# tomershay100/mp3-steganography-lib

Measured on AMD Instinct MI355X. Metric: MP3 frames/sec (decode+re-encode) @44.1kHz stereo 128kbps, 1→8 GPU, higher is better.
Workload: dtype f64 (decode) / int32 (encode); 1 GPU; 10000-frame full decode->stego-embed->re-encode pipeline per MI355X (BASELINE configs[2]); MP3 main data + side info resident in HBM, MP3 frames out; the message cursor chain is decided and the serial chains of the rate loop are checked on the device inside every step; frames_per_gpu=10000, channels=2, message_bits=536, chain_verdict_units_to_redo=0, message_variant_entries=1874, parallelism=frames sharded over 1 GPU(s), no collective

## Files before the change

### mp3-steganography-lib_amd/csrc/k_decode_stream.hpp

```cpp
#pragma once
#ifndef MP3S_ST_CLOCKS
#define MP3S_ST_CLOCKS 0
#endif
#if MP3S_ST_CLOCKS
__device__ uint32_t g_st_clocks[4096 * 8];
extern "C" __attribute__((visibility("default"))) int mp3s_debug_st_clocks(uint32_t *out)
{
    (void)hipDeviceSynchronize();
    return (int)hipMemcpyFromSymbol(out, HIP_SYMBOL(g_st_clocks), sizeof(uint32_t) * 4096 * 8);
}
#endif

namespace mp3s {

constexpr int ST_WAVES = 4;
constexpr int ST_P43_N = 512;

struct StShared {
    double pow2q[POW2Q_N];
    double pow2h[POW2H_N];
    uint32_t side[ST_WAVES][2][18];
    double exp2f[ST_WAVES][2][64];
    double exp1f[ST_WAVES][2][4];
    double win[4][36];
    double tail[ST_WAVES][18][64];
    double p43[2 * ST_P43_N];
    double cx[16][32], wt[16][32];
};

__device__ __forceinline__ double st_requant_line(const DevTables &tab, StShared &sh, int wave, const int16_t *__restrict__ is, int g, int c, int sr, int s)
{
    const uint8_t *gb = reinterpret_cast<const uint8_t *>(sh.side[wave][c]);
    const int bt = gb[2] & 3, mixed = gb[3] ? 1 : 0;
    const int cse = bt == 2 ? 1 : (mixed ? 2 : 0);
    const int sbs = (s * 3641) >> 16;
    const uint32_t m = tab.rq_map[sr][cse][sbs][s - 18 * sbs];
    const int x = is[((long)g * 2 + c) * 576 + s];
    uint32_t ax = (uint32_t)(x < 0 ? -x : x);
    ax = ax < (uint32_t)POW43_N ? ax : (uint32_t)(POW43_N - 1);
    const double a = tab.pow43[ax];
    const double sa = x < 0 ? -a : a;
    return (sa * sh.exp1f[wave][c][m >> 6]) * sh.exp2f[wave][c][m & 63];
}

__device__ __forceinline__ double st_row_dot16(double t, const double (&c)[16])
{
    double x = 0.0;
    asm("s_nop 4\n\t"
        "v_fmac_f64_dpp %0, %1, %2 row_newbcast:0 row_mask:0xf bank_mask:0xf\n\t"
        "v_fmac_f64_dpp %0, %1, %3 row_newbcast:1 row_mask:0xf bank_mask:0xf\n\t"
        "v_fmac_f64_dpp %0, %1, %4 row_newbcast:2 row_mask:0xf bank_mask:0xf\n\t"
        "v_fmac_f64_dpp %0, %1, %5 row_newbcast:3 row_mask:0xf bank_mask:0xf\n\t"
        "v_fmac_f64_dpp %0, %1, %6 row_newbcast:4 row_mask:0xf bank_mask:0xf\n\t"
        "v_fmac_f64_dpp %0, %1, %7 row_newbcast:5 row_mask:0xf bank_mask:0xf\n\t"
        "v_fmac_f64_dpp %0, %1, %8 row_newbcast:6 row_mask:0xf bank_mask:0xf\n\t"
        "v_fmac_f64_dpp %0, %1, %9 row_newbcast:7 row_mask:0xf bank_mask:0xf\n\t"
        "v_fmac_f64_dpp %0, %1, %10 row_newbcast:8 row_mask:0xf bank_mask:0xf\n\t"
        "v_fmac_f64_dpp %0, %1, %11 row_newbcast:9 row_mask:0xf bank_mask:0xf\n\t"
        "v_fmac_f64_dpp %0, %1, %12 row_newbcast:10 row_mask:0xf bank_mask:0xf\n\t"
        "v_fmac_f64_dpp %0, %1, %13 row_newbcast:11 row_mask:0xf bank_mask:0xf\n\t"
        "v_fmac_f64_dpp %0, %1, %14 row_newbcast:12 row_mask:0xf bank_mask:0xf\n\t"
        "v_fmac_f64_dpp %0, %1, %15 row_newbcast:13 row_mask:0xf bank_mask:0xf\n\t"
        "v_fmac_f64_dpp %0, %1, %16 row_newbcast:14 row_mask:0xf bank_mask:0xf\n\t"
        "v_fmac_f64_dpp %0, %1, %17 row_newbcast:15 row_mask:0xf bank_mask:0xf"
        : "+v"(x)
        : "v"(t), "v"(c[0]), "v"(c[1]), "v"(c[2]), "v"(c[3]), "v"(c[4]), "v"(c[5]), "v"(c[6]), "v"(c[7]), "v"(c[8]), "v"(c[9]), "v"(c[10]),
          "v"(c[11]), "v"(c[12]), "v"(c[13]), "v"(c[14]), "v"(c[15]));
    return x;
}

template <int NCH, bool F32, bool MARGIN = false>
__global__ __launch_bounds__(ST_WAVES * 64, 2) void k_dec_stream(
    const int16_t *__restrict__ is, const mp3s_granule_si *__restrict__ si, const mp3s_frame_hdr *__restrict__ hdr,
    int n_granules, int run, int n_halo, void *__restrict__ pcm_out, int sf_base, double eps_scale,
    uint2 *__restrict__ fix_list, int32_t *__restrict__ fix_count,
    double *__restrict__ mg_x = nullptr, double *__restrict__ mg_eps = nullptr, long mg_base = 0, long mg_cap = 0)
{
    __shared__ StShared sh;
    const int wave = __builtin_amdgcn_readfirstlane(threadIdx.x >> 6), lane = threadIdx.x & 63;
#if MP3S_ST_CLOCKS
    const unsigned long long ck_start = __builtin_readcyclecounter();
    unsigned long long ck_req = 0, ck_rows = 0, ck_syn = 0, ck_setup = 0;
#endif
    for (int i = threadIdx.x; i < POW2Q_N; i += blockDim.x) sh.pow2q[i] = c_tab.pow2q[i];
    if (threadIdx.x < POW2H_N) sh.pow2h[threadIdx.x] = c_tab.pow2h[threadIdx.x];
    if (threadIdx.x < 144) (&sh.win[0][0])[threadIdx.x] = (&c_tab.sine_block[0][0])[threadIdx.x];
    for (int i = threadIdx.x; i < 2 * ST_P43_N; i += blockDim.x) {
        const int x = i - ST_P43_N;
        sh.p43[i] = x < 0 ? -c_tab.pow43[-x] : c_tab.pow43[x];
    }
    for (int i = threadIdx.x; i < 512; i += blockDim.x) {
        sh.cx[i >> 5][i & 31] = c_tab.stream_cx[i & 31][i >> 5];
        sh.wt[i >> 5][i & 31] = c_tab.stream_taps[F32 ? 0 : 1][i & 31][i >> 5];
    }
    __syncthreads();
    const int ga = (xcd_tile() * ST_WAVES + wave) * run;
    if (ga >= n_granules) return;

    const int ch = lane >> 5, sb = lane & 31;
    const bool live = ch < NCH;
    const uint32_t sgn_odd = (sb & 1) ? 0x80000000u : 0u;
    auto flip = [&](double x) { return __hiloint2double(__double2hiint(x) ^ (int)sgn_odd, __double2loint(x)); };
    int addr_a, addr_b;
    {
        const int ka = sb <= 15 ? 16 + sb : (sb == 16 ? 0 : 48 - sb);
        const int kb = sb <= 15 ? 16 - sb : sb - 16;
        auto holder = [&](int k) { return (ch << 5) + ((k & 1) ? (k >> 1) : 16 + (k >> 1)); };
        addr_a = holder(ka) * 4; addr_b = holder(kb) * 4;
    }
    const uint32_t sgn_lo = sb < 16 ? 0x80000000u : 0u;
    const double eps_k = (2.0 * c_tab.synth_eps_a + c_tab.synth_eps_g + 2.0 * c_tab.synth_eps_x * c_tab.synth_xbound) * eps_scale;
    const double xb_k = 2.0 * c_tab.synth_xbound;
    const long halo_slots = (long)n_halo * 36;
    typedef double __attribute__((address_space(3))) lds_f64;
    lds_f64 *const tl = (lds_f64 *)reinterpret_cast<double *>(&sh.tail[wave][0][lane]);

    double acc[18];
#pragma unroll
    for (int i = 0; i < 18; i++) acc[i] = 0.0;
    double gm1 = 0.0, gm2 = 0.0;
    const int s_a = [&] { const uint32_t sf = hdr[ga >> 1].stream_first; return sf > (uint32_t)sf_base ? (int)(sf - (uint32_t)sf_base) * 2 : 0; }();
    bool fresh = true;
    GranIn next_in = {};
    bool have_next = false;

    const int gi0 = ga - 2 >= s_a ? -2 : (ga - 1 >= s_a ? -1 : 0);
    mp3s_frame_hdr fh = hdr[(ga + gi0) >> 1];
    int sr_map = fh.sr_idx < 3 ? fh.sr_idx : 0;
    uint32_t mwl[5];
#pragma unroll
    for (int k = 0; k < 5; k++) mwl[k] = reinterpret_cast<const uint32_t *>(c_tab.rq_map[sr_map][0][sb])[k];
#if MP3S_ST_CLOCKS
    ck_setup = __builtin_readcyclecounter() - ck_start;
#endif
#pragma unroll 1
    for (int gi = gi0; gi < run; gi++) {
        const int g = ga + gi;
        if (g >= n_granules) break;
#if MP3S_ST_CLOCKS
        const unsigned long long ck_a = __builtin_readcyclecounter();
#endif
        const int first_gran = fh.stream_first > (uint32_t)sf_base ? (int)(fh.stream_first - (uint32_t)sf_base) * 2 : 0;
        const int sr = fh.sr_idx < 3 ? fh.sr_idx : 0;
        const bool ms = fh.ms_stereo != 0;
        fh = hdr[(g + 1 < n_granules ? g + 1 : g) >> 1];
        if (g == first_gran) fresh = true;
        if (fresh) {
#pragma unroll
            for (int i = 0; i < 18; i++) { tl[i * 64] = 0.0; acc[i] = 0.0; }
            gm1 = gm2 = 0.0;
            fresh = false;
        }
        const bool tail_only = gi == -2;
        const bool emit = gi >= 0;
        int zoff = 0;
        asm volatile("" : "+s"(zoff));
        const DevTables &tab = *reinterpret_cast<const DevTables *>(reinterpret_cast<const char *>(&c_tab) + zoff);
        const double(*C12)[6] = tab.imdct_cos12;

        double v[18];
        int bt, cse;
        const GranIn in = have_next ? next_in : dec_fetch(is, si, g, NCH, lane);
        bool quick;
        uint32_t w0, w1;
        {
            const uint32_t d0a = (uint32_t)__builtin_amdgcn_readlane((int)in.side, 0), d1a = (uint32_t)__builtin_amdgcn_readlane((int)in.side, 1);
            const uint32_t d0b = (uint32_t)__builtin_amdgcn_readlane((int)in.side, 18), d1b = (uint32_t)__builtin_amdgcn_readlane((int)in.side, 19);
            auto is_long = [](uint32_t d0) { return ((d0 >> 16) & 3u) != 2u && (d0 >> 24) == 0u; };
            quick = is_long(d0a) && (NCH == 1 || is_long(d0b));
            w0 = ch ? d0b : d0a; w1 = ch ? d1b : d1a;
            uint32_t hi_bits = 0;
#pragma unroll
            for (int k = 0; k < 9; k++) {
                uint32_t t;
                asm("v_pk_add_u16 %0, %1, %2" : "=v"(t) : "v"(in.xw[k]), "v"(0x02000200u));
                hi_bits |= t;
            }
            quick = quick && __ballot((hi_bits & 0xfc00fc00u) != 0) == 0;
        }
        if (quick && sr != sr_map) {
            sr_map = sr;
#pragma unroll
            for (int k = 0; k < 5; k++) mwl[k] = reinterpret_cast<const uint32_t *>(tab.rq_map[sr][0][sb])[k];
        }
        if (quick) {
            bt = (int)((w0 >> 16) & 3u); cse = 0;
            const int gg = (int)(w0 & 0xffu), mult2 = ((w0 >> 8) & 0xffu) ? 2 : 1, preflag = (w1 & 0xffu) ? 1 : 0;
            double *e2 = sh.exp2f[wave][ch];
            const int bsrc = ((ch ? 18 : 0) + 2 + (sb >> 2)) * 4;
            const uint32_t sfw = (uint32_t)__builtin_amdgcn_ds_bpermute(bsrc, (int)in.side);
            if (sb < 22) {
                const int pt = sb < 11 || sb > 20 ? 0 : (int)((0x2333221111ull >> ((sb - 11) * 4)) & 15);
                const int k2 = mult2 * ((int)((sfw >> ((sb & 3) * 8)) & 15u) + preflag * pt);
                e2[sb] = sh.pow2h[k2 < POW2H_N ? k2 : POW2H_N - 1];
            }
            const double e1 = sh.pow2q[gg - 210 - POW2Q_MIN];
            __builtin_amdgcn_s_waitcnt(0xc07f);
            __builtin_amdgcn_wave_barrier();
#pragma unroll
            for (int k = 0; k < 18; k++) {
                const uint32_t xwk = in.xw[k >> 1];
                const int x = (k & 1) ? (int)xwk >> 16 : (int)(int16_t)xwk;
                const double sa = sh.p43[x + ST_P43_N];
                uint32_t i2;
                asm("v_bfe_u32 %0, %1, %2, 6" : "=v"(i2) : "v"(mwl[k >> 2]), "n"((k & 3) * 8));
                v[k] = (sa * e1) * e2[i2];
            }
            if (ms && NCH == 2) {
#pragma unroll
                for (int k = 0; k < 18; k++) {
                    const double o = shfl_xor_f64(v[k], 32);
                    v[k] = ch == 0 ? (v[k] + o) / tab.sqrt2 : (o - v[k]) / tab.sqrt2;
                }
            }
        } else {
            const uint32_t sd0a = (uint32_t)__builtin_amdgcn_readlane((int)in.side, 0), sd0b = (uint32_t)__builtin_amdgcn_readlane((int)in.side, 18);
            auto case_of = [](uint32_t d0) { return ((d0 >> 16) & 3u) == 2u ? 1 : ((d0 >> 24) ? 2 : 0); };
            const int cse_a = case_of(sd0a), cse_b = NCH == 2 ? case_of(sd0b) : cse_a;
            if (cse_a == cse_b && cse_a != 0) {
                dec_requant_tables(sh, wave, in, NCH, lane, bt, cse);
                const uint32_t *srcw = reinterpret_cast<const uint32_t *>(tab.reorder_src[sr] + sb * 18);
                uint32_t sw[9];
#pragma unroll
                for (int k = 0; k < 9; k++) sw[k] = srcw[k];
#pragma unroll
                for (int k = 0; k < 18; k++) {
                    const int s = (int)(int16_t)(sw[k >> 1] >> ((k & 1) * 16));
                    v[k] = s >= 0 && live ? st_requant_line(tab, sh, wave, is, g, ch, sr, s) : 0.0;
                }
                if (ms && NCH == 2) {
#pragma unroll
                    for (int k = 0; k < 18; k++) {
                        const double o = shfl_xor_f64(v[k], 32);
                        v[k] = ch == 0 ? (v[k] + o) / tab.sqrt2 : (o - v[k]) / tab.sqrt2;
                    }
                }
                cse = -1;
            } else
                dec_requant_ms(tab, sh, wave, v, in, sr, ms, NCH, lane, bt, cse);
        }
        if (cse > 0) {
            const uint32_t *srcw = reinterpret_cast<const uint32_t *>(tab.reorder_src[sr] + sb * 18);
            uint32_t sw[9];
#pragma unroll
            for (int k = 0; k < 9; k++) sw[k] = srcw[k];
#pragma unroll
            for (int k = 0; k < 18; k++) {
                const int s = (int)(int16_t)(sw[k >> 1] >> ((k & 1) * 16));
                double x = 0.0;
                if (s >= 0 && live) {
                    x = st_requant_line(tab, sh, wave, is, g, ch, sr, s);
                    if (ms && NCH == 2) {
                        const double o = st_requant_line(tab, sh, wave, is, g, ch ^ 1, sr, s);
                        x = ch == 0 ? (x + o) / tab.sqrt2 : (o - x) / tab.sqrt2;
                    }
                }
                v[k] = x;
            }
        } else if (cse == 0) {
#pragma unroll
            for (int i = 0; i < 8; i++) {
                const double nlo = dpp_f64<0x138>(v[17 - i]);
                const double nhi = dpp_f64<0x130>(v[i]);
                const double cs = tab.alias_cs[i], ca = tab.alias_ca[i];
                const double lo = v[i] * cs + nlo * ca;
                const double hi = v[17 - i] * cs - nhi * ca;
                v[i] = sb >= 1 ? lo : v[i];
                v[17 - i] = sb <= 30 ? hi : v[17 - i];
            }
        }
        double eps_t = 0.0;
        bool safe = true;
        if (!F32) {
            double s = 0.0;
#pragma unroll
            for (int k = 0; k < 18; k++) s += fabs(v[k]);
            s += dpp_f64<0xB1>(s);
            s += dpp_f64<0x4E>(s);
            s += dpp_f64<0x141>(s);
            s += dpp_f64<0x140>(s);
            const double o = __hiloint2double(__builtin_amdgcn_ds_swizzle(__double2hiint(s), 0x401f), __builtin_amdgcn_ds_swizzle(__double2loint(s), 0x401f));
            const double gc = s + o;
            double gx = gc > gm1 ? gc : gm1;
            gx = gx > gm2 ? gx : gm2;
            if (!(gx >= 0.0)) gx = __builtin_inf();
            eps_t = eps_k * gx;
            safe = __ballot(!(xb_k * gx < 2147483000.0)) == 0;
            gm2 = gm1; gm1 = gc;
        }

#if MP3S_ST_CLOCKS
        const unsigned long long ck_b = __builtin_readcyclecounter();
        ck_req += ck_b - ck_a;
#endif
        double S[18];
        if (bt != 2) {
            const double *wl = sh.win[bt];
            double p[9], q[9];
            {
                const Row18s r = load_row18s(tab.imdct_rot, 0);
#pragma unroll
                for (int k = 0; k < 9; k++) {
                    const double c = 2 * k < 8 ? r.a[2 * k] : (2 * k < 16 ? r.b[2 * k - 8] : r.c[2 * k - 16]);
                    const double sn = 2 * k + 1 < 8 ? r.a[2 * k + 1] : (2 * k + 1 < 16 ? r.b[2 * k + 1 - 8] : r.c[2 * k + 1 - 16]);
                    p[k] = __builtin_fma(v[17 - k], sn, v[k] * c);
                    q[k] = __builtin_fma(v[17 - k], c, -(v[k] * sn));
                }
            }
            struct StageIn { Row18s c; double w[4], t[4]; };
            auto stage_in = [&](auto mc) {
                constexpr int m = decltype(mc)::value;
                StageIn in;
                in.c = load_row18s(tab.imdct_pq, m);
#pragma unroll
                for (int h = 0; h < 2; h++) {
                    const int n = h == 0 ? 2 * m : 2 * m - 1;
                    in.w[2 * h] = in.w[2 * h + 1] = in.t[2 * h] = in.t[2 * h + 1] = 0.0;
                    if (n < 0 || n > 17) continue;
                    if (n >= 9) {
                        const int i = n - 9;
                        in.w[2 * h] = wl[i]; in.w[2 * h + 1] = wl[17 - i];
                        in.t[2 * h] = tl[i * 64]; in.t[2 * h + 1] = tl[(17 - i) * 64];
                    } else {
                        const int i = 26 - n;
                        in.w[2 * h] = wl[i]; in.w[2 * h + 1] = wl[53 - i];
                    }
                }
                return in;
            };
            auto stage = [&](auto mc, const StageIn &in) {
                constexpr int m = decltype(mc)::value;
                double P = 0.0, Q = 0.0;
#pragma unroll
                for (int k = 0; k < 9; k++) {
                    const double cp = k < 8 ? in.c.a[k] : in.c.b[0];
                    const double cq = k < 7 ? in.c.b[1 + k] : in.c.c[k - 7];
                    if (m != 9) P = __builtin_fma(p[k], cp, P);
                    if (m != 0) Q = __builtin_fma(q[k], cq, Q);
                }
#pragma unroll
                for (int h = 0; h < 2; h++) {
                    const int n = h == 0 ? 2 * m : 2 * m - 1;
                    if (n < 0 || n > 17) continue;
                    const double y = h == 0 ? P + Q : P - Q;
                    if (n >= 9) {
                        const int i = n - 9;
                        double xa = y * in.w[2 * h] + in.t[2 * h];
                        double xb = -y * in.w[2 * h + 1] + in.t[2 * h + 1];
                        if (i & 1) xa = flip(xa);
                        if ((17 - i) & 1) xb = flip(xb);
                        S[i] = xa; S[17 - i] = xb;
                    } else {
                        const int i = 26 - n;
                        tl[(i - 18) * 64] = -y * in.w[2 * h];
                        tl[(35 - i) * 64] = -y * in.w[2 * h + 1];
                    }
                }
            };
#define MP3S_ST_STAGE(M, MNEXT)                                                                 \
            {                                                                                   \
                __builtin_amdgcn_s_waitcnt(0xc07f);                                             \
                __builtin_amdgcn_sched_barrier(0);                                              \
                const StageIn nxt = stage_in(std::integral_constant<int, MNEXT>{});             \
                __builtin_amdgcn_sched_barrier(0);                                              \
                stage(std::integral_constant<int, M>{}, cur);                                   \
                __builtin_amdgcn_sched_barrier(0);                                              \
                cur = nxt;                                                                      \
            }
            StageIn cur;
            if (!tail_only) {
                cur = stage_in(std::integral_constant<int, 9>{});
                MP3S_ST_STAGE(9, 8) MP3S_ST_STAGE(8, 7) MP3S_ST_STAGE(7, 6) MP3S_ST_STAGE(6, 5) MP3S_ST_STAGE(5, 4)
            } else
                cur = stage_in(std::integral_constant<int, 4>{});
            MP3S_ST_STAGE(4, 3) MP3S_ST_STAGE(3, 2) MP3S_ST_STAGE(2, 1) MP3S_ST_STAGE(1, 0) MP3S_ST_STAGE(0, 0)
#undef MP3S_ST_STAGE
        } else {
            typedef double dvec4 __attribute__((ext_vector_type(4)));
            struct Row6 { dvec4 a; dvec2 b; double s; };
            auto load_row6 = [&](int j) { Row6 r; r.a = *reinterpret_cast<const dvec4 *>(C12[j]); r.b = *reinterpret_cast<const dvec2 *>(C12[j] + 4); r.s = tab.sine_block[2][j]; return r; };
            double hold[6], tn[6];
#pragma unroll
            for (int i = 0; i < 6; i++) { double x = 0.0 + (double)tl[i * 64]; if (i & 1) x = flip(x); S[i] = x; }
            Row6 cur = load_row6(0);
#pragma unroll
            for (int j = 0; j < 12; j++) {
                const Row6 nxt = load_row6(j < 11 ? j + 1 : 11);
                const double pj = tl[(6 + j) * 64];
                __builtin_amdgcn_sched_barrier(0);
                double a0 = 0.0, a1 = 0.0, a2 = 0.0;
#pragma unroll
                for (int k = 0; k < 6; k++) {
                    const double c = k < 4 ? cur.a[k] : cur.b[k - 4];
                    a0 += v[k] * c; a1 += v[6 + k] * c; a2 += v[12 + k] * c;
                }
                a0 = a0 * cur.s; a1 = a1 * cur.s; a2 = a2 * cur.s;
                if (j < 6) {
                    double x = a0 + pj;
                    if ((6 + j) & 1) x = flip(x);
                    S[6 + j] = x;
                    hold[j] = a1;
                    tn[j] = a2;
                } else {
                    double x = (a0 + hold[j - 6]) + pj;
                    if ((6 + j) & 1) x = flip(x);
                    S[6 + j] = x;
                    tn[j - 6] = a1 + tn[j - 6];
                    tl[j * 64] = a2;
                    tl[(6 + j) * 64] = 0.0;
                }
                __builtin_amdgcn_sched_barrier(0);
                cur = nxt;
            }
#pragma unroll
            for (int i = 0; i < 6; i++) tl[i * 64] = tn[i];
        }
        have_next = gi + 1 < run && g + 1 < n_granules;
        if (have_next) next_in = dec_fetch(is, si, g + 1, NCH, lane);
#if MP3S_ST_CLOCKS
        const unsigned long long ck_c = __builtin_readcyclecounter();
        ck_rows += ck_c - ck_b;
#endif
        if (tail_only) continue;

        const long t0 = (long)g * 18;
        const bool store = emit && t0 >= halo_slots;
        int16_t *const o16 = reinterpret_cast<int16_t *>(pcm_out) + ((t0 - halo_slots) * 32 + sb) * NCH + ch;
        float *const o32 = reinterpret_cast<float *>(pcm_out) + ((t0 - halo_slots) * 32 + sb) * NCH + ch;
        double cx[16], wt[16];
#pragma unroll
        for (int j = 0; j < 16; j++) { cx[j] = sh.cx[j][sb]; wt[j] = sh.wt[j][sb]; }
        auto mirror = [&](double s) { return __hiloint2double(__builtin_amdgcn_ds_swizzle(__double2hiint(s), 0x7c1f), __builtin_amdgcn_ds_swizzle(__double2loint(s), 0x7c1f)); };
        auto xsum = [&](double s, double m) {
            const double ms2 = __hiloint2double(__double2hiint(m) ^ (int)sgn_lo, __double2loint(m));
            return st_row_dot16(s + ms2, cx);
        };
        double mir = mirror(S[0]);
        double X = xsum(S[0], mir);
        int a_lo = __builtin_amdgcn_ds_bpermute(addr_a, __double2loint(X)), a_hi = __builtin_amdgcn_ds_bpermute(addr_a, __double2hiint(X));
        int b_lo = __builtin_amdgcn_ds_bpermute(addr_b, __double2loint(X)), b_hi = __builtin_amdgcn_ds_bpermute(addr_b, __double2hiint(X));
        mir = mirror(S[1]);
#pragma unroll
        for (int p = 0; p < 18; p++) {
            const double A = __hiloint2double(a_hi, a_lo), B = __hiloint2double(b_hi, b_lo);
            if (p < 17) {
                X = xsum(S[p + 1], mir);
                a_lo = __builtin_amdgcn_ds_bpermute(addr_a, __double2loint(X)); a_hi = __builtin_amdgcn_ds_bpermute(addr_a, __double2hiint(X));
                b_lo = __builtin_amdgcn_ds_bpermute(addr_b, __double2loint(X)); b_hi = __builtin_amdgcn_ds_bpermute(addr_b, __double2hiint(X));
                if (p < 16) mir = mirror(S[p + 2]);
            }
#pragma unroll
            for (int jj = 0; jj < 16; jj++) {
                const int q = (p + jj) % 18;
                const double val = (jj & 1) ? B : A;
                acc[q] = jj == 15 ? wt[15] * val : __builtin_fma(wt[jj], val, acc[q]);
            }
            const double x = acc[p];
            if (F32) {
                if (store && live) o32[p * 32 * NCH] = (float)x;
            } else {
                const double xi = rint(x);
                const double dist = fabs(x) - fmax(fabs(xi), 1.0);
                if (store) {
                    if (live) o16[p * 32 * NCH] = (int16_t)(int)x;
                    if (MARGIN && live) {
                        const long at = mg_base + ((t0 - halo_slots + p) * 32 + sb) * NCH + ch;
                        if (at >= 0 && at < mg_cap) { mg_x[at] = x; mg_eps[at] = safe ? eps_t : __builtin_inf(); }
                    }
                    unsigned long long m = safe ? __ballot(!(fabs(dist) > eps_t)) : ~0ull;
                    if (NCH == 1) m &= 0xffffffffull;
                    if (__builtin_expect(m != 0, 0)) {
                        if (lane == 0) {
                            const uint32_t m0 = (uint32_t)m, m1 = (uint32_t)(m >> 32);
                            const int n = (m0 != 0) + (m1 != 0);
                            int at = atomicAdd(fix_count, n);
                            if (m0) fix_list[at++] = make_uint2((uint32_t)(t0 + p), m0);
                            if (m1) fix_list[at] = make_uint2((uint32_t)(t0 + p) | 0x80000000u, m1);
                        }
                    }
                }
            }
        }
#if MP3S_ST_CLOCKS
        ck_syn += __builtin_readcyclecounter() - ck_c;
#endif
    }
#if MP3S_ST_CLOCKS
    if (lane == 0) {
        uint32_t *d = g_st_clocks + ((size_t)(xcd_tile() * ST_WAVES + wave) & 4095) * 8;
        d[0] = (uint32_t)ck_setup; d[1] = (uint32_t)ck_req; d[2] = (uint32_t)ck_rows; d[3] = (uint32_t)ck_syn;
        d[4] = (uint32_t)(__builtin_readcyclecounter() - ck_start);
    }
#endif
}

}
```

Before: 20.98 million frames/s.

## Overlap table staging with header/first-granule fetch and halve IMDCT stage FMAs via symmetry

```diff
diff --git a/mp3-steganography-lib_amd/csrc/k_decode_stream.hpp b/mp3-steganography-lib_amd/csrc/k_decode_stream.hpp
--- a/mp3-steganography-lib_amd/csrc/k_decode_stream.hpp
+++ b/mp3-steganography-lib_amd/csrc/k_decode_stream.hpp
@@ -15,6 +15,20 @@
 
 constexpr int ST_WAVES = 4;
 constexpr int ST_P43_N = 512;
+typedef double dvec4s __attribute__((ext_vector_type(4), aligned(8)));
+
+struct StHdr {
+    uint32_t w, stream_first;
+    __device__ __forceinline__ int sr_idx() const { return (int)(w & 0xffu); }
+    __device__ __forceinline__ int ms_stereo() const { return (int)((w >> 16) & 0xffu); }
+};
+static_assert(sizeof(mp3s_frame_hdr) == 8 && offsetof(mp3s_frame_hdr, sr_idx) == 0 && offsetof(mp3s_frame_hdr, ms_stereo) == 2 && offsetof(mp3s_frame_hdr, stream_first) == 4,
+              "StHdr reads mp3s_frame_hdr as two dwords");
+__device__ __forceinline__ StHdr st_hdr(const mp3s_frame_hdr *__restrict__ hdr, int frame)
+{
+    const uint2 d = reinterpret_cast<const uint2 *>(hdr)[frame];
+    return StHdr{d.x, d.y};
+}
 
 struct StShared {
     double pow2q[POW2Q_N];
@@ -82,23 +96,60 @@
     const unsigned long long ck_start = __builtin_readcyclecounter();
     unsigned long long ck_req = 0, ck_rows = 0, ck_syn = 0, ck_setup = 0;
 #endif
-    for (int i = threadIdx.x; i < POW2Q_N; i += blockDim.x) sh.pow2q[i] = c_tab.pow2q[i];
-    if (threadIdx.x < POW2H_N) sh.pow2h[threadIdx.x] = c_tab.pow2h[threadIdx.x];
-    if (threadIdx.x < 144) (&sh.win[0][0])[threadIdx.x] = (&c_tab.sine_block[0][0])[threadIdx.x];
-    for (int i = threadIdx.x; i < 2 * ST_P43_N; i += blockDim.x) {
-        const int x = i - ST_P43_N;
-        sh.p43[i] = x < 0 ? -c_tab.pow43[-x] : c_tab.pow43[x];
-    }
-    for (int i = threadIdx.x; i < 512; i += blockDim.x) {
-        sh.cx[i >> 5][i & 31] = c_tab.stream_cx[i & 31][i >> 5];
-        sh.wt[i >> 5][i & 31] = c_tab.stream_taps[F32 ? 0 : 1][i & 31][i >> 5];
+    const int ga = (xcd_tile() * ST_WAVES + wave) * run;
+    const int gq = ga < n_granules ? ga : n_granules - 1;
+    const StHdr fh_a = st_hdr(hdr, gq >> 1), fh_b = st_hdr(hdr, gq >= 2 ? (gq - 2) >> 1 : 0);
+    const int ch = lane >> 5, sb = lane & 31;
+    const bool live = ch < NCH;
+    int gi0, sr_map;
+    StHdr fh;
+    uint32_t mwl[5];
+    GranIn next_in;
+    {
+        constexpr int NT = ST_WAVES * 64, NQ = (POW2Q_N + NT - 1) / NT, NP = 2 * ST_P43_N / NT, NC = 512 / NT;
+        static_assert(POW2H_N <= NT && 144 <= NT && 2 * ST_P43_N % NT == 0 && 512 % NT == 0, "one table element per thread and trip");
+        const int t = threadIdx.x;
+        double rq[NQ], rp[NP], rc[NC], rw[NC];
+#pragma unroll
+        for (int j = 0; j < NQ; j++) rq[j] = c_tab.pow2q[t + j * NT < POW2Q_N ? t + j * NT : POW2Q_N - 1];
+        const double rh = c_tab.pow2h[t < POW2H_N ? t : POW2H_N - 1];
+        const double rs = (&c_tab.sine_block[0][0])[t < 144 ? t : 143];
+#pragma unroll
+        for (int j = 0; j < NP; j++) {
+            const int x = t + j * NT - ST_P43_N;
+            rp[j] = c_tab.pow43[x < 0 ? -x : x];
+        }
+#pragma unroll
+        for (int j = 0; j < NC; j++) {
+            const int i = t + j * NT;
+            rc[j] = c_tab.stream_cx[i & 31][i >> 5];
+            rw[j] = c_tab.stream_taps[F32 ? 0 : 1][i & 31][i >> 5];
+        }
+        __builtin_amdgcn_sched_barrier(0);
+        const int s_a = fh_a.stream_first > (uint32_t)sf_base ? (int)(fh_a.stream_first - (uint32_t)sf_base) * 2 : 0;
+        gi0 = gq - 2 >= s_a ? -2 : (gq - 1 >= s_a ? -1 : 0);
+        fh = ((gq + gi0) >> 1) == (gq >> 1) ? fh_a : fh_b;
+        sr_map = fh.sr_idx() < 3 ? fh.sr_idx() : 0;
+#pragma unroll
+        for (int k = 0; k < 5; k++) mwl[k] = reinterpret_cast<const uint32_t *>(c_tab.rq_map[sr_map][0][sb])[k];
+        next_in = dec_fetch(is, si, gq + gi0, NCH, lane);
+        __builtin_amdgcn_sched_barrier(0);
+#pragma unroll
+        for (int j = 0; j < NQ; j++) if (t + j * NT < POW2Q_N) sh.pow2q[t + j * NT] = rq[j];
+        if (t < POW2H_N) sh.pow2h[t] = rh;
+        if (t < 144) (&sh.win[0][0])[t] = rs;
+#pragma unroll
+        for (int j = 0; j < NP; j++) sh.p43[t + j * NT] = t + j * NT < ST_P43_N ? -rp[j] : rp[j];
+#pragma unroll
+        for (int j = 0; j < NC; j++) {
+            const int i = t + j * NT;
+            sh.cx[i >> 5][i & 31] = rc[j];
+            sh.wt[i >> 5][i & 31] = rw[j];
+        }
     }
     __syncthreads();
-    const int ga = (xcd_tile() * ST_WAVES + wave) * run;
     if (ga >= n_granules) return;
 
-    const int ch = lane >> 5, sb = lane & 31;
-    const bool live = ch < NCH;
     const uint32_t sgn_odd = (sb & 1) ? 0x80000000u : 0u;
     auto flip = [&](double x) { return __hiloint2double(__double2hiint(x) ^ (int)sgn_odd, __double2loint(x)); };
     int addr_a, addr_b;
@@ -119,17 +170,7 @@
 #pragma unroll
     for (int i = 0; i < 18; i++) acc[i] = 0.0;
     double gm1 = 0.0, gm2 = 0.0;
-    const int s_a = [&] { const uint32_t sf = hdr[ga >> 1].stream_first; return sf > (uint32_t)sf_base ? (int)(sf - (uint32_t)sf_base) * 2 : 0; }();
     bool fresh = true;
-    GranIn next_in = {};
-    bool have_next = false;
-
-    const int gi0 = ga - 2 >= s_a ? -2 : (ga - 1 >= s_a ? -1 : 0);
-    mp3s_frame_hdr fh = hdr[(ga + gi0) >> 1];
-    int sr_map = fh.sr_idx < 3 ? fh.sr_idx : 0;
-    uint32_t mwl[5];
-#pragma unroll
-    for (int k = 0; k < 5; k++) mwl[k] = reinterpret_cast<const uint32_t *>(c_tab.rq_map[sr_map][0][sb])[k];
 #if MP3S_ST_CLOCKS
     ck_setup = __builtin_readcyclecounter() - ck_start;
 #endif
@@ -141,9 +182,9 @@
         const unsigned long long ck_a = __builtin_readcyclecounter();
 #endif
         const int first_gran = fh.stream_first > (uint32_t)sf_base ? (int)(fh.stream_first - (uint32_t)sf_base) * 2 : 0;
-        const int sr = fh.sr_idx < 3 ? fh.sr_idx : 0;
-        const bool ms = fh.ms_stereo != 0;
-        fh = hdr[(g + 1 < n_granules ? g + 1 : g) >> 1];
+        const int sr = fh.sr_idx() < 3 ? fh.sr_idx() : 0;
+        const bool ms = fh.ms_stereo() != 0;
+        fh = st_hdr(hdr, (g + 1 < n_granules ? g + 1 : g) >> 1);
         if (g == first_gran) fresh = true;
         if (fresh) {
 #pragma unroll
@@ -160,7 +201,7 @@
 
         double v[18];
         int bt, cse;
-        const GranIn in = have_next ? next_in : dec_fetch(is, si, g, NCH, lane);
+        const GranIn in = next_in;
         bool quick;
         uint32_t w0, w1;
         {
@@ -296,9 +337,10 @@
         double S[18];
         if (bt != 2) {
             const double *wl = sh.win[bt];
-            double p[9], q[9];
+            double ap[4], dp[4], aq[4], dq[4], p4, q4;
             {
                 const Row18s r = load_row18s(tab.imdct_rot, 0);
+                double p[9], q[9];
 #pragma unroll
                 for (int k = 0; k < 9; k++) {
                     const double c = 2 * k < 8 ? r.a[2 * k] : (2 * k < 16 ? r.b[2 * k - 8] : r.c[2 * k - 16]);
@@ -306,12 +348,19 @@
                     p[k] = __builtin_fma(v[17 - k], sn, v[k] * c);
                     q[k] = __builtin_fma(v[17 - k], c, -(v[k] * sn));
                 }
-            }
-            struct StageIn { Row18s c; double w[4], t[4]; };
+#pragma unroll
+                for (int k = 0; k < 4; k++) {
+                    ap[k] = p[k] + p[8 - k]; dp[k] = p[k] - p[8 - k];
+                    aq[k] = q[k] + q[8 - k]; dq[k] = q[k] - q[8 - k];
+                }
+                p4 = p[4]; q4 = q[4];
+            }
+            struct StageIn { dvec4s c, s; double w[4], t[4]; };
             auto stage_in = [&](auto mc) {
                 constexpr int m = decltype(mc)::value;
                 StageIn in;
-                in.c = load_row18s(tab.imdct_pq, m);
+                in.c = *reinterpret_cast<const dvec4s *>(tab.imdct_pq[m]);
+                in.s = *reinterpret_cast<const dvec4s *>(tab.imdct_pq[m] + 9);
 #pragma unroll
                 for (int h = 0; h < 2; h++) {
                     const int n = h == 0 ? 2 * m : 2 * m - 1;
@@ -330,13 +379,13 @@
             };
             auto stage = [&](auto mc, const StageIn &in) {
                 constexpr int m = decltype(mc)::value;
-                double P = 0.0, Q = 0.0;
-#pragma unroll
-                for (int k = 0; k < 9; k++) {
-                    const double cp = k < 8 ? in.c.a[k] : in.c.b[0];
-                    const double cq = k < 7 ? in.c.b[1 + k] : in.c.c[k - 7];
-                    if (m != 9) P = __builtin_fma(p[k], cp, P);
-                    if (m != 0) Q = __builtin_fma(q[k], cq, Q);
+                constexpr bool even = (m & 1) == 0;
+                double P = even ? ((m >> 1) & 1 ? -p4 : p4) : 0.0;
+                double Q = even ? 0.0 : ((m >> 1) & 1 ? -q4 : q4);
+#pragma unroll
+                for (int k = 0; k < 4; k++) {
+                    if (m != 9) P = __builtin_fma(even ? ap[k] : dp[k], in.c[k], P);
+                    if (m != 0) Q = __builtin_fma(even ? dq[k] : aq[k], in.s[k], Q);
                 }
 #pragma unroll
                 for (int h = 0; h < 2; h++) {
@@ -415,8 +464,7 @@
 #pragma unroll
             for (int i = 0; i < 6; i++) tl[i * 64] = tn[i];
         }
-        have_next = gi + 1 < run && g + 1 < n_granules;
-        if (have_next) next_in = dec_fetch(is, si, g + 1, NCH, lane);
+        if (gi + 1 < run && g + 1 < n_granules) next_in = dec_fetch(is, si, g + 1, NCH, lane);
 #if MP3S_ST_CLOCKS
         const unsigned long long ck_c = __builtin_readcyclecounter();
         ck_rows += ck_c - ck_b;
```

Result: faster. 21.62 million frames/s, median of 6 (+3.0%).
